# LUMC/kPAL

Hardware: AMD Instinct MI355X
Metric: Gbases/s k-mer counted (k=12, 150bp synthetic) (higher is better)
Workload: dtype int64

## Files before the change

### kpal_amd/csrc/kpal_device.hpp

```cpp
#pragma once
#include <hip/hip_runtime.h>
#include <stdint.h>

namespace kpal {

__host__ __device__ inline uint64_t mix64(uint64_t x)
{
    uint64_t z = x + 0x9E3779B97F4A7C15ULL;
    z = (z ^ (z >> 30)) * 0xBF58476D1CE4E5B9ULL;
    z = (z ^ (z >> 27)) * 0x94D049BB133111EBULL;
    return z ^ (z >> 31);
}

__host__ __device__ inline uint64_t revcomp(uint64_t x, int k)
{
    uint64_t y = ~x;
#if defined(__HIP_DEVICE_COMPILE__)
    y = __brevll(y);
#else
    y = ((y >> 1) & 0x5555555555555555ULL) | ((y & 0x5555555555555555ULL) << 1);
    y = ((y >> 2) & 0x3333333333333333ULL) | ((y & 0x3333333333333333ULL) << 2);
    y = ((y >> 4) & 0x0F0F0F0F0F0F0F0FULL) | ((y & 0x0F0F0F0F0F0F0F0FULL) << 4);
    y = ((y >> 8) & 0x00FF00FF00FF00FFULL) | ((y & 0x00FF00FF00FF00FFULL) << 8);
    y = ((y >> 16) & 0x0000FFFF0000FFFFULL) | ((y & 0x0000FFFF0000FFFFULL) << 16);
    y = (y >> 32) | (y << 32);
#endif
    y = ((y >> 1) & 0x5555555555555555ULL) | ((y & 0x5555555555555555ULL) << 1);
    return y >> (64 - 2 * k);
}

__device__ __forceinline__ void classify4(uint32_t w, uint32_t &t, uint32_t &nz)
{
    t = ((w >> 1) ^ (w >> 2)) & 0x03030303u;
    const uint32_t expect = __builtin_amdgcn_perm(0u, 0x54474341u , t);
    const uint32_t x = (w & 0xDFDFDFDFu) ^ expect;
    nz = (((x & 0x7F7F7F7Fu) + 0x7F7F7F7Fu) | x) & 0x80808080u;
}

template <int SH>
__device__ __forceinline__ uint32_t shl_or(uint32_t a, uint32_t b)
{
    uint32_t r;
    asm("v_lshl_or_b32 %0, %1, %2, %3" : "=v"(r) : "v"(a), "n"(SH), "v"(b));
    return r;
}

__device__ __forceinline__ uint32_t codes_to_top_byte(uint32_t t)
{
    const uint32_t x = shl_or<10>(t, t);
    return shl_or<20>(x, x);
}

__device__ __forceinline__ uint32_t flags_to_top_byte(uint32_t m)
{
    const uint32_t x = shl_or<9>(m, m);
    return shl_or<18>(x, x);
}

__device__ __forceinline__ void encode4(uint32_t w, uint32_t &code8, uint32_t &bad4)
{
    uint32_t t, nz;
    classify4(w, t, nz);
    code8 = codes_to_top_byte(t) >> 24;
    bad4 = flags_to_top_byte(nz >> 7) >> 24;
}

struct Chunk {
    uint32_t codes;
    uint32_t bad;
};

__device__ __forceinline__ Chunk encode16(uint4 v)
{
    uint32_t t0, t1, t2, t3, z0, z1, z2, z3;
    classify4(v.x, t0, z0);
    classify4(v.y, t1, z1);
    classify4(v.z, t2, z2);
    classify4(v.w, t3, z3);
    Chunk r;
#if defined(KPAL_ENCODE_SHIFTS)
    const uint32_t c0 = codes_to_top_byte(t0), c1 = codes_to_top_byte(t1), c2 = codes_to_top_byte(t2), c3 = codes_to_top_byte(t3);
    const uint32_t c01 = __builtin_amdgcn_perm(c0, c1, 0x07030000u);
    const uint32_t c23 = __builtin_amdgcn_perm(c2, c3, 0x07030000u);
    const uint32_t f01 = flags_to_top_byte((z0 >> 3) | (z1 >> 7));
    const uint32_t f23 = flags_to_top_byte((z2 >> 3) | (z3 >> 7));
    r.codes = __builtin_amdgcn_perm(c01, c23, 0x07060302u);
    r.bad = __builtin_amdgcn_perm(f01, f23, 0x0c0c0703u);
#else
    constexpr uint32_t kDigits = 0x01041040u;
    const uint32_t d0 = __builtin_amdgcn_udot4(t0, kDigits, 0u, false), d1 = __builtin_amdgcn_udot4(t1, kDigits, 0u, false);
    const uint32_t d2 = __builtin_amdgcn_udot4(t2, kDigits, 0u, false), d3 = __builtin_amdgcn_udot4(t3, kDigits, 0u, false);
    r.codes = (d0 << 24) | ((d1 << 16) | ((d2 << 8) | d3));
    constexpr uint32_t kHigh = 0x10204080u, kLow = 0x01020408u;
    const uint32_t f01 = __builtin_amdgcn_udot4(z1, kLow, __builtin_amdgcn_udot4(z0, kHigh, 0u, false), false);
    const uint32_t f23 = __builtin_amdgcn_udot4(z3, kLow, __builtin_amdgcn_udot4(z2, kHigh, 0u, false), false);
    r.bad = (f01 << 1) | (f23 >> 7);
#endif
    return r;
}

struct Span {
    const uint4 *base;
    uint64_t lo;
    uint64_t hi;
    uint64_t emit_from;
    uint64_t nchunks;
};

__device__ __forceinline__ uint4 fetch_chunk(const Span &s, int64_t c)
{
    if (c < 0 || (uint64_t)c >= s.nchunks) return make_uint4(0u, 0u, 0u, 0u);
    return s.base[c];
}

__device__ __forceinline__ void range_fix(const Span &s, int64_t c, Chunk &r)
{
    if (c < 0 || (uint64_t)c >= s.nchunks) {
        r.codes = 0;
        r.bad = 0xFFFFu;
        return;
    }
    const uint64_t p0 = (uint64_t)c * 16;
    if (p0 < s.lo || p0 + 16 > s.hi) {
        const uint32_t a = s.lo > p0 ? (uint32_t)(s.lo - p0) : 0u;
        const uint32_t b = s.hi < p0 + 16 ? (uint32_t)(s.hi > p0 ? s.hi - p0 : 0) : 16u;
        const uint32_t in_range = (a < b) ? (((1u << (16 - a)) - 1u) & ~((1u << (16 - b)) - 1u)) : 0u;
        r.bad |= ~in_range & 0xFFFFu;
    }
}

__device__ __forceinline__ Chunk load_chunk(const Span &s, int64_t c)
{
    Chunk r = encode16(fetch_chunk(s, c));
    range_fix(s, c, r);
    return r;
}

template <int K>
__device__ __forceinline__ uint32_t emit_mask(uint32_t prev_bad, uint32_t cur_bad)
{
    uint32_t b = (prev_bad << 16) | cur_bad;
    uint32_t s = b;
    int have = 1;
#pragma unroll
    for (int step = 1; step < 32; step <<= 1) {
        if (have * 2 <= K) {
            s |= s >> have;
            have *= 2;
        }
    }
    if (have < K) s |= s >> (K - have);
    return ~s & 0xFFFFu;
}

__device__ __forceinline__ uint32_t emit_mask_rt(int k, uint32_t prev_bad, uint32_t cur_bad)
{
    uint32_t b = (prev_bad << 16) | cur_bad;
    uint32_t s = b;
    int have = 1;
    while (have * 2 <= k) {
        s |= s >> have;
        have *= 2;
    }
    if (have < k) s |= s >> (k - have);
    return ~s & 0xFFFFu;
}

__device__ __forceinline__ uint32_t emit_from_mask(const Span &s, int64_t c)
{
    const uint64_t p0 = (uint64_t)c * 16;
    if (s.emit_from <= p0) return 0xFFFFu;
    if (s.emit_from >= p0 + 16) return 0u;
    return (1u << (16 - (uint32_t)(s.emit_from - p0))) - 1u;
}

__device__ __forceinline__ uint32_t from_left_lane(uint32_t v, uint32_t lane0_value)
{
    return (uint32_t)__builtin_amdgcn_update_dpp((int)lane0_value, (int)v, 0x138 , 0xF, 0xF, false);
}

template <int K, bool EDGE>
__device__ __forceinline__ void wave_step(const Span &s, int64_t c, Chunk &carry, uint64_t &window,
                                          uint32_t &mask)
{
    Chunk cur;
    if constexpr (EDGE) cur = load_chunk(s, c);
    else cur = encode16(s.base[c]);
    const uint32_t pc = from_left_lane(cur.codes, carry.codes);
    const uint32_t pb = from_left_lane(cur.bad, carry.bad);
    carry.codes = __builtin_amdgcn_readlane(cur.codes, 63);
    carry.bad = __builtin_amdgcn_readlane(cur.bad, 63);
    window = ((uint64_t)pc << 32) | cur.codes;
    mask = emit_mask<K>(pb, cur.bad);
    if constexpr (EDGE) mask &= emit_from_mask(s, c);
}

template <int K>
__device__ __forceinline__ void encode_step(const Span &s, uint64_t step, const uint4 raw, Chunk &carry,
                                            uint64_t &window, uint32_t &mask, bool edge)
{
    const int lane = threadIdx.x & 63;
    const int64_t c = (int64_t)(step * 64 + lane);
    Chunk cur = encode16(raw);
    if (edge) range_fix(s, c, cur);
    const uint32_t pc = from_left_lane(cur.codes, carry.codes);
    const uint32_t pb = from_left_lane(cur.bad, carry.bad);
    carry.codes = __builtin_amdgcn_readlane(cur.codes, 63);
    carry.bad = __builtin_amdgcn_readlane(cur.bad, 63);
    window = ((uint64_t)pc << 32) | cur.codes;
    mask = emit_mask<K>(pb, cur.bad);
    if (edge) mask &= emit_from_mask(s, c);
}

__device__ __forceinline__ bool interior_steps(const Span &s, uint64_t step0, uint64_t step1)
{
    return step0 * 64 >= 1 && (step0 * 64 - 1) * 16 >= s.lo && step1 * 64 * 16 <= s.hi && s.emit_from <= step0 * 64 * 16;
}

template <int K>
__device__ __forceinline__ void encode_step(const Span &s, uint64_t step, const uint4 raw, Chunk &carry,
                                            uint64_t &window, uint32_t &mask)
{
    encode_step<K>(s, step, raw, carry, window, mask, !interior_steps(s, step, step + 1));
}

__device__ __forceinline__ bool interior_range(const Span &s, uint64_t c0, uint64_t c1)
{
    return c0 >= 1 && (c0 - 1) * 16 >= s.lo && c1 * 16 <= s.hi && s.emit_from <= c0 * 16;
}

template <int K>
__device__ __forceinline__ uint32_t kmer_at(uint64_t window, int j)
{
    constexpr uint64_t M = (K >= 16) ? 0xFFFFFFFFULL : ((1ULL << (2 * K)) - 1ULL);
    return (uint32_t)((window >> (2 * (15 - j))) & M);
}

template <int K>
__device__ __forceinline__ void part_step(const Span &s, uint64_t step, Chunk &carry, uint64_t &window, uint32_t &mask)
{
    const int lane = threadIdx.x & 63;
    if (interior_range(s, step * 64, step * 64 + 64)) wave_step<K, false>(s, (int64_t)(step * 64 + lane), carry, window, mask);
    else wave_step<K, true>(s, (int64_t)(step * 64 + lane), carry, window, mask);
}

__device__ __forceinline__ void lds_barrier()
{
    asm volatile("s_waitcnt lgkmcnt(0)\n\ts_barrier" ::: "memory");
}

}
```

### kpal_amd/csrc/quad_kernels.hpp

```cpp
#pragma once
#include <type_traits>

#include "kpal_device.hpp"
#include "quad2_index.hpp"
#include "quad_plan.hpp"

namespace kpal {

constexpr int kQuadSpillCap = 2048;
constexpr int kQuadDummyWords = 4;

template <int K>
struct QuadCfg {
    static_assert(K >= 8 && K <= 16, "quads: k = 8..16");
    static constexpr bool kTwoLevel = K >= 13;
    static constexpr bool kStaged = K >= 12;
    static constexpr int kCoarseBits = kTwoLevel ? 2 * K - 22 : 0;
    static constexpr int kCoarse = 1 << kCoarseBits;
    static constexpr int kRep = kTwoLevel ? (kCoarse >= 256 ? 1 : 256 / kCoarse) : 1;
    static constexpr int kBucketBits = kTwoLevel ? 9 : (K == 12 ? 11 : 9);
    static constexpr int kHistBuckets = 1 << kBucketBits;
    static constexpr int kBuckets = kTwoLevel ? kCoarse * kRep : (1 << kBucketBits);
    static constexpr int kLowBits = kTwoLevel ? 13 : 2 * K - kBucketBits;
    static constexpr int kFormBins = 1 << kLowBits;
    static constexpr int kSlots = kQuadRowWords / kBuckets;
    static constexpr int kRecordBytes = kSlots * 4;
#if defined(KPAL_QUAD_ITEM4)
    static constexpr bool kItem3 = false;
#else
    static constexpr bool kItem3 = !kTwoLevel && K == 12;
#endif
    static constexpr int kItems = kItem3 ? (kSlots / 4) * 5 : kSlots;
#if defined(KPAL_QUAD_NO_PAIR)
    static constexpr bool kPairRows = false;
#else
    static constexpr bool kPairRows = !kTwoLevel && kRecordBytes == 64;
#endif
    static constexpr int kScrBits = (kLowBits - 6) < 4 ? (kLowBits - 6) : 4;
    static constexpr uint64_t kXMask = (1ull << (2 * K + 6)) - 1ull;
    static constexpr uint32_t kLowMask = (1u << kLowBits) - 1u;
    __host__ __device__ static constexpr uint32_t smask(uint32_t t)
    {
        return kScrBits > 0 ? (((t << (kBucketBits - kScrBits)) | t) & (uint32_t)((1 << kBucketBits) - 1)) : 0u;
    }
    __host__ __device__ static constexpr uint32_t smask1(uint32_t t) { return (kCoarseBits > 4 ? ((t << (kCoarseBits - 4)) ^ t) : t) & (uint32_t)(kCoarse - 1); }
};

static_assert(Quad2Index<13>::smask(11) == QuadCfg<13>::smask(11) && Quad2Index<16>::smask(5) == QuadCfg<16>::smask(5) &&
                  Quad2Index<13>::smask1(9) == QuadCfg<13>::smask1(9) && Quad2Index<14>::smask1(13) == QuadCfg<14>::smask1(13) &&
                  Quad2Index<15>::smask1(7) == QuadCfg<15>::smask1(7) && Quad2Index<16>::smask1(15) == QuadCfg<16>::smask1(15) &&
                  Quad2Index<15>::CB == QuadCfg<15>::kCoarseBits &&
                  ((Quad2Index<12>::smask1(13) << 9) | Quad2Index<12>::smask(13)) == QuadCfg<12>::smask(13) &&
                  ((Quad2Index<12>::smask1(6) << 9) | Quad2Index<12>::smask(6)) == QuadCfg<12>::smask(6),
              "quad2_index.hpp restates the scramble masks of QuadCfg");

template <int K>
__device__ __forceinline__ void quad_split(uint64_t x, uint32_t m4, uint32_t lane, uint32_t &row, uint32_t &item)
{
    using C = QuadCfg<K>;
    const uint32_t low = (uint32_t)x & C::kLowMask;
    const uint32_t hi6 = (uint32_t)(x >> (2 * K));
    if constexpr (C::kTwoLevel) {
        const uint32_t fine = ((uint32_t)x >> 13) & 511u;
        const uint32_t coarse = (uint32_t)(x >> 22) & (uint32_t)(C::kCoarse - 1);
        row = (coarse ^ C::smask1(low >> 9)) * C::kRep + (lane & (uint32_t)(C::kRep - 1));
        item = (hi6 << 26) | (fine << 17) | (low << 4) | m4;
    } else {
        const uint32_t b = ((uint32_t)x >> C::kLowBits) & (uint32_t)(C::kBuckets - 1);
        row = b ^ C::smask(low >> (C::kLowBits - C::kScrBits));
        item = (hi6 << (C::kLowBits + 4)) | (low << 4) | m4;
    }
}

template <int K, int LEVEL = 1>
__device__ __forceinline__ uint32_t quad_kmer(uint32_t row, uint32_t item, int i, uint32_t coarse = 0)
{
    using C = QuadCfg<K>;
    uint64_t x;
    if constexpr (LEVEL == 2) {
        const uint32_t low = (item >> 4) & 8191u, hi6 = item >> 17, t = low >> 9;
        x = ((uint64_t)hi6 << (2 * K)) | ((uint64_t)(coarse ^ C::smask1(t)) << 22) | ((uint64_t)(row ^ C::smask(t)) << 13) | low;
    } else if constexpr (C::kTwoLevel) {
        const uint32_t low = (item >> 4) & 8191u, fine = (item >> 17) & 511u, hi6 = item >> 26, t = low >> 9;
        x = ((uint64_t)hi6 << (2 * K)) | ((uint64_t)((row / C::kRep) ^ C::smask1(t)) << 22) | ((uint64_t)fine << 13) | low;
    } else {
        const uint32_t low = (item >> 4) & C::kLowMask;
        const uint32_t hi6 = item >> (C::kLowBits + 4);
        const uint32_t b = row ^ C::smask(low >> (C::kLowBits - C::kScrBits));
        x = ((uint64_t)hi6 << (2 * K)) | ((uint64_t)b << C::kLowBits) | low;
    }
    return (uint32_t)((x >> (6 - 2 * i)) & ((1ull << (2 * K)) - 1ull));
}

struct QuadPacked {
    uint32_t a, b, c;
};
__device__ __forceinline__ QuadPacked quad_pack3(const uint4 &v)
{
    QuadPacked r;
    r.a = v.x | (v.y << 23);
    r.b = (v.y >> 9) | (v.z << 14);
    r.c = (v.z >> 18) | (v.w << 5);
    return r;
}
__device__ __forceinline__ uint4 quad_unpack3(uint32_t a, uint32_t b, uint32_t c)
{
    uint4 v;
    v.x = a & 0x7FFFFFu;
    v.y = __builtin_amdgcn_alignbit(b, a, 23) & 0x7FFFFFu;
    v.z = __builtin_amdgcn_alignbit(c, b, 14) & 0x7FFFFFu;
    v.w = (c >> 5) & 0x7FFFFFu;
    return v;
}

struct QuadSpill {
    uint32_t row, item;
};

struct QuadHot {
    unsigned long long key;
    uint32_t count, pad;
};
constexpr int kQuadHotEntries = 256;

struct TableSink {
    unsigned long long *table;
    unsigned long long *list;
    uint32_t *count;
    uint32_t cap;
    uint32_t *overflow;
};

struct TableOnly {
    unsigned long long *table;
};

__device__ __forceinline__ void sink_add(const TableOnly &sink, uint64_t index, unsigned long long n) { atomicAdd(&sink.table[index], n); }

struct TableSinkRef {
    const TableSink *p;
};

__device__ __forceinline__ void sink_add(const TableSink &sink, uint64_t index, unsigned long long n);
__device__ __forceinline__ void sink_add(const TableSinkRef &ref, uint64_t index, unsigned long long n) { sink_add(*ref.p, index, n); }

__device__ __forceinline__ void sink_add(const TableSink &sink, uint64_t index, unsigned long long n)
{
    if (sink.table) {
        atomicAdd(&sink.table[index], n);
    } else {
        const uint32_t at = atomicAdd(sink.count, 1u);
        if (at < sink.cap) sink.list[at] = ((unsigned long long)index << 32) | (n & 0xFFFFFFFFull);
        else *sink.overflow = 1u;
    }
}

__device__ __forceinline__ uint32_t quad_hot_hash(uint32_t row, uint32_t item)
{
    return ((item >> 4) * 0x9E3779B1u + row * 0x85EBCA6Bu) >> 24;
}

template <typename SINK>
__device__ __attribute__((noinline)) void quad_hot_age(const SINK table, QuadHot *hot)
{
    const QuadHot h = hot[threadIdx.x];
    if (h.key >> 63) {
        if (h.count == h.pad) {
            sink_add(table, (uint64_t)(h.key & 0x7FFFFFFFFFFFFFFFull), (unsigned long long)h.count);
            hot[threadIdx.x] = QuadHot{0ull, 0u, 0u};
        } else {
            hot[threadIdx.x].pad = h.count;
        }
    }
}

template <typename SINK>
__device__ __forceinline__ void quad_kmer_add(const SINK table, QuadHot *hot, uint64_t index, uint32_t n)
{
#if defined(KPAL_AB_DIRECT_NO_TABLE)
    return;
#endif
    const unsigned long long key = (1ull << 63) | (unsigned long long)index;
    const uint32_t h = ((uint32_t)index * 0x9E3779B1u + (uint32_t)(index >> 32)) >> 24;
    bool done = false;
#pragma unroll 1
    for (uint32_t pr = 0; pr < 4u && !done; ++pr) {
        const uint32_t slot = (h + pr) & (uint32_t)(kQuadHotEntries - 1);
        unsigned long long cur = hot[slot].key;
        if (cur == 0ull) {
            cur = atomicCAS(&hot[slot].key, 0ull, key);
            if (cur == 0ull) cur = key;
        }
        if (cur == key) {
            atomicAdd(&hot[slot].count, n);
            done = true;
        }
    }
    if (!done) sink_add(table, index, (unsigned long long)n);
}

template <int K, int LEVEL = 1, typename SINK = TableOnly, bool COUNTED = false, bool KMERS = false>
__device__ __forceinline__ void quad_items_direct_body(bool active, uint32_t row, uint32_t item, const SINK table, QuadHot *hot, uint32_t coarse = 0,
                                                       uint32_t cnt = 1u)
{
    const uint32_t mult = COUNTED ? cnt : 1u;
    const int lane = threadIdx.x & 63;
    auto kmer_add = [&](uint64_t index, uint32_t n) {
        if constexpr (KMERS) quad_kmer_add<SINK>(table, hot, index, n);
        else sink_add(table, index, (unsigned long long)n);
    };
    auto to_table = [&](uint32_t r, uint32_t it, uint32_t n) {
#pragma unroll
        for (int i = 0; i < 4; ++i)
            if ((it >> (3 - i)) & 1u) sink_add(table, quad_kmer<K, LEVEL>(r, it, i, coarse), (unsigned long long)n);
    };
    unsigned long long todo = __builtin_amdgcn_ballot_w64(active);
    for (int round = 0; round < 8 && todo; ++round) {
        const int src = __ffsll((long long)todo) - 1;
        const uint32_t hot_row = (uint32_t)__builtin_amdgcn_readlane(row, src);
        const uint32_t hot_item = (uint32_t)__builtin_amdgcn_readlane(item, src);
        const unsigned long long same = __builtin_amdgcn_ballot_w64(active && row == hot_row && item == hot_item) & todo;
        uint32_t n = (uint32_t)__popcll(same);
        if constexpr (COUNTED) {
            n = 0;
#pragma unroll
            for (uint32_t v = 1; v <= 4u; ++v) n += v * (uint32_t)__popcll(same & __builtin_amdgcn_ballot_w64(cnt == v));
        }
        const unsigned long long key = ((unsigned long long)hot_row << 32) | hot_item;
        const uint32_t slot = (quad_hot_hash(hot_row, hot_item) + (uint32_t)(lane & 3)) & (uint32_t)(kQuadHotEntries - 1);
        const unsigned long long seen = lane < 4 ? hot[slot].key : ~0ull;
        const unsigned long long hit = __builtin_amdgcn_ballot_w64(seen == key);
        if (hit) {
            if (lane == __ffsll((long long)hit) - 1) atomicAdd(&hot[slot].count, n);
        } else {
            const unsigned long long free_slots = __builtin_amdgcn_ballot_w64(seen == 0ull);
            bool placed = false;
            if (n >= 2u && free_slots) {
                const int who = __ffsll((long long)free_slots) - 1;
                const unsigned long long old = lane == who ? atomicCAS(&hot[slot].key, 0ull, key) : 1ull;
                placed = __builtin_amdgcn_ballot_w64(lane == who && (old == 0ull || old == key)) != 0ull;
                if (placed && lane == who) atomicAdd(&hot[slot].count, n);
            }
            if constexpr (KMERS) {
                if (!placed && lane < 4 && ((hot_item >> (3 - lane)) & 1u)) kmer_add(quad_kmer<K, LEVEL>(hot_row, hot_item, lane, coarse), n);
            } else {
                if (!placed && lane == src) to_table(hot_row, hot_item, n);
            }
        }
        todo &= ~same;
    }
    if ((todo >> lane) & 1ull) {
        const unsigned long long key = ((unsigned long long)row << 32) | item;
        const uint32_t h = quad_hot_hash(row, item);
        bool done = false;
#pragma unroll
        for (int pr = 0; pr < 4 && !done; ++pr) {
            const uint32_t slot = (h + (uint32_t)pr) & (uint32_t)(kQuadHotEntries - 1);
            if (hot[slot].key == key) {
                atomicAdd(&hot[slot].count, mult);
                done = true;
            }
        }
        if (!done) to_table(row, item, mult);
    }
}

template <int K, int LEVEL = 1, typename SINK = TableOnly, bool KM = false>
__device__ __attribute__((noinline)) void quad_items_direct(bool active, uint32_t row, uint32_t item, const SINK table, QuadHot *hot, uint32_t coarse = 0)
{
    quad_items_direct_body<K, LEVEL, SINK, false, KM>(active, row, item, table, hot, coarse);
}

template <int K, typename SINK>
__device__ __attribute__((noinline)) void quad_items_direct_counted(uint32_t cnt, uint32_t row, uint32_t item, const SINK table, QuadHot *hot)
{
    quad_items_direct_body<K, 1, SINK, true, true>(cnt != 0u, row, item, table, hot, 0u, cnt);
}

template <int K, bool DIRECT = false, int LEVEL = 1, int N = 4, typename SINK = TableOnly, bool KM = false>
__device__ __forceinline__ uint32_t quad_place(uint32_t *rows, uint32_t *pos, QuadSpill *spill, uint32_t *spill_n, uint32_t cap,
                                               const uint32_t (&row)[N], const uint32_t (&item)[N], const SINK &table,
                                               QuadHot *hot, uint32_t coarse = 0)
{
    using C = typename std::conditional<LEVEL == 2, QuadCfg<11>, QuadCfg<K>>::type;
    constexpr uint32_t RB = (uint32_t)C::kSlots * 4u;
    constexpr bool ITEM3 = LEVEL == 1 && C::kItem3;
    uint32_t riders = 0;
    uint32_t off[N];
#pragma unroll
    for (int q = 0; q < N; ++q) off[q] = atomicAdd(&pos[row[q]], (item[q] & 15u) ? 4u : 0u);
    uint32_t over = 0;
#pragma unroll
    for (int q = 0; q < N; ++q) {
        const bool counted = (item[q] & 15u) != 0u;
        if constexpr (ITEM3) {
            const bool normal = off[q] < RB;
            const bool rider = !normal && off[q] < RB + RB / 4;
            if (counted && normal) atomicOr(reinterpret_cast<uint32_t *>(reinterpret_cast<char *>(rows) + row[q] * RB + off[q]), item[q]);
            riders |= (counted && rider) ? (1u << q) : 0u;
            over |= (counted && !normal && !rider) ? (1u << q) : 0u;
        } else {
            const bool fits = off[q] < RB;
            const uint32_t at = row[q] * RB + off[q];
            *reinterpret_cast<uint32_t *>(reinterpret_cast<char *>(rows) + ((counted && fits) ? at : (uint32_t)kQuadRowWords * 4u)) = item[q];
            over |= (counted && !fits) ? (1u << q) : 0u;
        }
    }
#if defined(KPAL_AB_SCATTER_NO_RIDER)
    riders = 0;
#endif
#if defined(KPAL_AB_SCATTER_NO_SPILL)
    over = 0;
#endif
    if constexpr (ITEM3) {
        if (__any(riders != 0u)) {
#pragma unroll
            for (int q = 0; q < N; ++q)
                if ((riders >> q) & 1u) {
                    uint32_t *p = reinterpret_cast<uint32_t *>(reinterpret_cast<char *>(rows) + row[q] * RB + (off[q] - RB) * 4u);
#if defined(KPAL_AB_RIDER_OR)
                    atomicOr(p, item[q] << 24);
                    atomicOr(p + 1, (item[q] << 16) & 0xFF000000u);
                    atomicOr(p + 2, (item[q] << 8) & 0xFF000000u);
#else
                    reinterpret_cast<unsigned char *>(p)[3] = (unsigned char)item[q];
                    reinterpret_cast<unsigned char *>(p)[7] = (unsigned char)(item[q] >> 8);
                    reinterpret_cast<unsigned char *>(p)[11] = (unsigned char)(item[q] >> 16);
#endif
                }
        }
    }
    if (__builtin_expect(__any(over != 0u), 0)) {
#if defined(KPAL_QUAD_NO_CARRY)
        constexpr bool direct = true;
#else
        constexpr bool direct = DIRECT;
#endif
#if defined(KPAL_AB_SPILL_LANE)
        if constexpr (!direct) {
            uint32_t at[N];
#pragma unroll
            for (int q = 0; q < N; ++q) at[q] = cap;
            if (over) {
#pragma unroll
                for (int q = 0; q < N; ++q)
                    if ((over >> q) & 1u) at[q] = atomicAdd(spill_n, 1u);
            }
            uint32_t unlisted = 0;
#pragma unroll
            for (int q = 0; q < N; ++q) {
                const bool ov = (over >> q) & 1u;
                if (ov && at[q] < cap) spill[at[q]] = QuadSpill{row[q], item[q]};
                unlisted |= (ov && at[q] >= cap) ? (1u << q) : 0u;
            }
            if (__builtin_expect(__any(unlisted != 0u), 0)) {
#pragma unroll
                for (int q = 0; q < N; ++q)
                    if (__any((unlisted >> q) & 1u)) quad_items_direct<K, LEVEL, SINK, KM>((unlisted >> q) & 1u, row[q], item[q], table, hot, coarse);
            }
            return over;
        }
#endif
        uint32_t base = 0;
        bool list_full = true;
        unsigned long long bq[N];
#pragma unroll
        for (int q = 0; q < N; ++q) bq[q] = __builtin_amdgcn_ballot_w64((over >> q) & 1u);
        if constexpr (!direct) {
            uint32_t total = 0;
#pragma unroll
            for (int q = 0; q < N; ++q) total += (uint32_t)__popcll(bq[q]);
            uint32_t got = 0;
            if ((threadIdx.x & 63u) == 0u) got = atomicAdd(spill_n, total);
            base = (uint32_t)__builtin_amdgcn_readfirstlane((int)got);
            list_full = base + total > cap;
        }
#pragma unroll
        for (int q = 0; q < N; ++q) {
            if (bq[q] == 0ull) continue;
            const bool ov = (over >> q) & 1u;
            bool listed = false;
            if constexpr (!direct) {
                const unsigned long long b = bq[q];
                const uint32_t at = base + __builtin_amdgcn_mbcnt_hi((uint32_t)(b >> 32), __builtin_amdgcn_mbcnt_lo((uint32_t)b, 0u));
                listed = ov && at < cap;
                if (listed) spill[at] = QuadSpill{row[q], item[q]};
                base += (uint32_t)__popcll(b);
            }
            if (list_full && __any(ov && !listed)) quad_items_direct<K, LEVEL, SINK, KM>(ov && !listed, row[q], item[q], table, hot, coarse);
        }
    }
    return over;
}

template <int K, int CARRY, int LEVEL = 1, typename SINK = TableOnly, bool KM = false>
__device__ __forceinline__ void quad_place_carried(uint32_t *rows, uint32_t *pos, QuadSpill *spill, uint32_t *spill_n, uint32_t cap,
                                                   const uint32_t (&carry_row)[CARRY], uint32_t (&carry_item)[CARRY],
                                                   const SINK &table, QuadHot *hot, uint32_t coarse = 0)
{
#pragma unroll
    for (int c = 0; c < CARRY; ++c) {
        const uint32_t r1[1] = {carry_row[c]};
        const uint32_t i1[1] = {carry_item[c]};
        if (__any(carry_item[c] != 0u)) {
            if (quad_place<K, true, LEVEL, 1, SINK, KM>(rows, pos, spill, spill_n, cap, r1, i1, table, hot, coarse) & 1u) carry_item[c] = 0;
        }
    }
}

template <int CARRY, int THREADS>
__device__ __forceinline__ void quad_take_carried(const QuadSpill *spill, uint32_t n, uint32_t (&carry_row)[CARRY],
                                                  uint32_t (&carry_item)[CARRY])
{
#pragma unroll
    for (int c = 0; c < CARRY; ++c) {
        const uint32_t e = threadIdx.x + (uint32_t)c * THREADS;
        carry_item[c] = 0;
        if (e < n) {
            carry_row[c] = spill[e].row;
            carry_item[c] = spill[e].item;
        }
    }
}

template <int STEPS>
__device__ __forceinline__ void quad_tile_priority(int st)
{
#if !defined(KPAL_QUAD_NO_PRIO)
    const int level = st * 4 / STEPS;
    if (st == 0 || level != (st - 1) * 4 / STEPS) {
        switch (level) {
        case 0: __builtin_amdgcn_s_setprio(3); break;
        case 1: __builtin_amdgcn_s_setprio(2); break;
        case 2: __builtin_amdgcn_s_setprio(1); break;
        default: __builtin_amdgcn_s_setprio(0); break;
        }
    }
#endif
}

__device__ __forceinline__ void quad_note_spill(uint32_t *__restrict__ error, uint32_t appended, uint32_t cap)
{
    if (threadIdx.x == 0 && appended) {
        atomicAdd(error + 2, min(appended, cap));
        if (appended > cap) atomicAdd(error + 3, appended - cap);
    }
}

template <int K>
__global__ __launch_bounds__(512) void quad_sample_kernel(Span s, uint64_t stride_steps, uint32_t steps, uint32_t *__restrict__ load)
{
    using C = QuadCfg<K>;
    constexpr int NFINE = C::kTwoLevel ? 512 : 0;
    constexpr int NCNT = C::kBuckets + NFINE + 1;
    __shared__ uint32_t cnt[NCNT];
    for (int i = threadIdx.x; i < NCNT; i += blockDim.x) cnt[i] = 0;
    __syncthreads();
    const int wave = threadIdx.x >> 6;
    const uint64_t total_steps = (s.nchunks + 63) / 64;
    const uint64_t first = (uint64_t)blockIdx.x * stride_steps + (uint64_t)wave * steps;
    if (first < total_steps) {
        Chunk carry = load_chunk(s, (int64_t)(first * 64) - 1);
        for (uint32_t st = 0; st < steps && first + st < total_steps; ++st) {
            uint64_t window;
            uint32_t mask;
            part_step<K>(s, first + st, carry, window, mask);
            uint32_t row[4], item[4];
#pragma unroll
            for (int q = 0; q < 4; ++q) {
                const uint64_t x = (window >> (24 - 8 * q)) & C::kXMask;
                quad_split<K>(x, (mask >> (12 - 4 * q)) & 15u, threadIdx.x & 63u, row[q], item[q]);
            }
            {
                const bool c01 = item[1] == item[0] && row[1] == row[0] && (item[1] & 15u) == 15u;
                const bool c23 = item[3] == item[2] && row[3] == row[2] && (item[3] & 15u) == 15u;
                const unsigned long long cand = __builtin_amdgcn_ballot_w64(c01 || c23);
                if (cand) {
                    const int src = __ffsll((long long)cand) - 1;
                    const uint32_t hot_item = (uint32_t)__builtin_amdgcn_readlane(c01 ? item[1] : item[3], src);
                    const uint32_t hot_row = (uint32_t)__builtin_amdgcn_readlane(c01 ? row[1] : row[3], src);
                    uint32_t n = 0;
#pragma unroll
                    for (int q = 0; q < 4; ++q) {
                        const bool m = item[q] == hot_item && row[q] == hot_row;
                        n += m ? 1u : 0u;
                        item[q] = m ? 0u : item[q];
                    }
                    if (n) atomicAdd(&cnt[NCNT - 1], n);
                }
            }
#pragma unroll
            for (int q = 0; q < 4; ++q) {
                atomicAdd(&cnt[row[q]], (item[q] & 15u) ? 1u : 0u);
                if constexpr (C::kTwoLevel) {
                    const uint32_t fine_row = ((item[q] >> 17) & 511u) ^ QuadCfg<11>::smask(((item[q] >> 4) & 8191u) >> 9);
                    atomicAdd(&cnt[C::kBuckets + fine_row], (item[q] & 15u) ? 1u : 0u);
                }
            }
        }
    }
    __syncthreads();
    for (int i = threadIdx.x; i < NCNT; i += blockDim.x)
        if (cnt[i]) atomicAdd(&load[i], cnt[i]);
}

__device__ __forceinline__ uint4 fetch_wave_step(const Span &s, uint64_t step, uint32_t lane16)
{
    if ((step + 1) * 64 <= s.nchunks)
        return *reinterpret_cast<const uint4 *>(reinterpret_cast<const char *>(s.base + step * 64) + lane16);
    return fetch_chunk(s, (int64_t)(step * 64 + (lane16 >> 4)));
}


template <int K, int WAVES, int STEPS, int DEPTH, typename SINK = TableOnly, bool REPEAT = false>
__global__ __launch_bounds__(WAVES * 64) void quad_scatter_kernel(Span s, uint64_t tiles_per_block, uint32_t *__restrict__ pool,
                                                                  uint32_t rounds_cap, uint32_t *__restrict__ nrounds,
                                                                  uint32_t *__restrict__ error, SINK sink_arg)
{
    using C = QuadCfg<K>;
    constexpr bool kLists = std::is_same<SINK, TableSink>::value;
    constexpr int S = C::kSlots, NB = C::kBuckets;
    constexpr int THREADS = WAVES * 64;
    constexpr int kQuadTileSteps = WAVES * STEPS;
    constexpr int CARRY = kQuadSpillCap / THREADS;
    constexpr uint32_t CAP = CARRY * THREADS;
    static_assert((WAVES == 8 || WAVES == 16) && STEPS % DEPTH == 0, "tile shape");
    __shared__ __attribute__((aligned(16))) uint32_t rows[kQuadRowWords + kQuadDummyWords];
    __shared__ __attribute__((aligned(16))) uint32_t pos[NB];
    __shared__ QuadSpill spill[kQuadSpillCap];
    __shared__ uint32_t spill_cnt[2];
    __shared__ QuadHot hot[kQuadHotEntries];
    __shared__ uint32_t direct_n;
    __shared__ TableSink sink_lds;
    using SINK2 = typename std::conditional<kLists, TableSinkRef, SINK>::type;
    SINK2 table;
    if constexpr (kLists) {
        if (threadIdx.x == 0) {
            TableSink t = sink_arg;
            if (t.list) {
                t.list += (size_t)blockIdx.x * t.cap;
                t.count = &direct_n;
            }
            sink_lds = t;
            direct_n = 0;
        }
        table = TableSinkRef{&sink_lds};
    } else {
        table = sink_arg;
    }
    const int wave = __builtin_amdgcn_readfirstlane((int)(threadIdx.x >> 6)), lane = threadIdx.x & 63;
    const uint32_t lane16 = (uint32_t)lane * 16u;
    for (int i = threadIdx.x; i < kQuadRowWords + kQuadDummyWords; i += THREADS) rows[i] = 0;
    for (int i = threadIdx.x; i < NB; i += THREADS) pos[i] = 0;
    for (int i = threadIdx.x; i < kQuadHotEntries; i += THREADS) hot[i] = QuadHot{0ull, 0u, 0u};
    if (threadIdx.x == 0) {
        spill_cnt[0] = 0;
        spill_cnt[1] = 0;
    }
    __syncthreads();
    const uint64_t total_steps = (s.nchunks + 63) / 64;
    auto tile_step = [&](uint64_t j) -> uint64_t { return ((j * gridDim.x + blockIdx.x) * WAVES + (uint64_t)wave) * STEPS; };
    auto tile_exists = [&](uint64_t j) -> bool { return j < tiles_per_block && (j * gridDim.x + blockIdx.x) * (uint64_t)kQuadTileSteps < total_steps; };
    uint4 raw[DEPTH];
    uint4 rawh;
    {
        const uint64_t f = tile_step(0);
#pragma unroll
        for (int st = 0; st < DEPTH; ++st) raw[st] = fetch_wave_step(s, f + st, lane16);
        rawh = fetch_chunk(s, (int64_t)(f * 64) - 1);
    }
    uint32_t round = 0;
    uint32_t carry_row[CARRY], carry_item[CARRY];
#pragma unroll
    for (int c = 0; c < CARRY; ++c) carry_row[c] = carry_item[c] = 0;
    constexpr int LPR = S / 4;
    constexpr int FI = kQuadRowWords / 4 / THREADS;
    static_assert(THREADS % LPR == 0, "a record is written by one wave");
    uint4 rec[FI];
    bool have_rec = false;
    constexpr int PAIR = C::kPairRows ? 2 : 1;
    static_assert((THREADS / LPR) % PAIR == 0, "row pairs are written by one instruction");
    const uint64_t row_bytes = (uint64_t)gridDim.x * rounds_cap * (uint64_t)(S * 4 * PAIR);
    const uint32_t thread_off = (uint32_t)((uint64_t)(threadIdx.x / (LPR * PAIR)) * row_bytes) + (threadIdx.x % (LPR * PAIR)) * 16u;
    auto store_rec = [&](int i) {
#if defined(KPAL_AB_POOL_FILL)
        if (i % 7 == 6) return;
#endif
        uint32_t o = thread_off;
        asm volatile("" : "+v"(o));
        const uint64_t sc = (uint64_t)(i * (THREADS / (LPR * PAIR))) * row_bytes + ((uint64_t)blockIdx.x * rounds_cap + (round - 1u)) * (uint64_t)(S * 4 * PAIR);
#if defined(KPAL_QUAD_NT)
        uint32_t *q = reinterpret_cast<uint32_t *>(reinterpret_cast<char *>(pool) + sc + o);
        __builtin_nontemporal_store(rec[i].x, q);
        __builtin_nontemporal_store(rec[i].y, q + 1);
        __builtin_nontemporal_store(rec[i].z, q + 2);
        __builtin_nontemporal_store(rec[i].w, q + 3);
#elif defined(KPAL_AB_SCATTER_NO_STORE)
        asm volatile("" ::"v"(rec[i].x ^ rec[i].y ^ rec[i].z ^ rec[i].w), "v"(o), "s"((uint32_t)sc));
#else
        *reinterpret_cast<uint4 *>(reinterpret_cast<char *>(pool) + sc + o) = rec[i];
#endif
    };
    auto store_rec_at = [&](int i, const uint4 &v) {
        const uint64_t sc = (uint64_t)i * (uint64_t)(THREADS / (LPR * PAIR)) * row_bytes + ((uint64_t)blockIdx.x * rounds_cap + (round - 1u)) * (uint64_t)(S * 4 * PAIR);
        *reinterpret_cast<uint4 *>(reinterpret_cast<char *>(pool) + sc + thread_off) = v;
    };
    for (uint64_t j = 0; tile_exists(j); ++j) {
        const uint64_t first = tile_step(j);
        const bool more = tile_exists(j + 1);
        const uint64_t fnext = tile_step(j + 1);
        const bool edge = !interior_steps(s, first, first + STEPS);
        const bool next_inside = more && (fnext + STEPS) * 64 <= s.nchunks;
        uint32_t *spill_n = &spill_cnt[j & 1];
        quad_place_carried<K, CARRY, 1, SINK2, REPEAT>(rows, pos, spill, spill_n, CAP, carry_row, carry_item, table, hot);
        Chunk carry = encode16(rawh);
        range_fix(s, (int64_t)(first * 64) - 1, carry);
        if (more) rawh = fetch_chunk(s, (int64_t)(fnext * 64) - 1);
#pragma unroll
        for (int st = 0; st < STEPS; ++st) {
            uint64_t window;
            uint32_t mask;
            quad_tile_priority<STEPS>(st);
            encode_step<K>(s, first + st, raw[st % DEPTH], carry, window, mask, edge);
            if (have_rec) {
#pragma unroll
                for (int i = st * (FI / STEPS); i < (st + 1) * (FI / STEPS); ++i) store_rec(i);
            }
            {
                uint32_t l16 = lane16;
                asm volatile("" : "+v"(l16));
                if (st + DEPTH < STEPS) raw[st % DEPTH] = fetch_wave_step(s, first + st + DEPTH, l16);
                else if (next_inside) raw[st % DEPTH] = *reinterpret_cast<const uint4 *>(reinterpret_cast<const char *>(s.base + (fnext + (st + DEPTH - STEPS)) * 64) + l16);
                else if (more) raw[st % DEPTH] = fetch_chunk(s, (int64_t)((fnext + (st + DEPTH - STEPS)) * 64 + (l16 >> 4)));
            }
            uint32_t row[4], item[4];
#pragma unroll
            for (int q = 0; q < 4; ++q) {
                const uint64_t x = (window >> (24 - 8 * q)) & C::kXMask;
                quad_split<K>(x, (mask >> (12 - 4 * q)) & 15u, (uint32_t)lane, row[q], item[q]);
            }
            bool place = true;
            if constexpr (REPEAT) {
                if (__builtin_expect(__any(item[1] == item[0] || item[3] == item[2]), 0)) {
                    const bool c01 = item[1] == item[0] && row[1] == row[0] && (item[1] & 15u) == 15u;
                    const bool c23 = item[3] == item[2] && row[3] == row[2] && (item[3] & 15u) == 15u;
                    const unsigned long long cand = __builtin_amdgcn_ballot_w64(c01 || c23);
                    if (cand) {
                        const int src = __ffsll((long long)cand) - 1;
                        const uint32_t hot_item = (uint32_t)__builtin_amdgcn_readlane(c01 ? item[1] : item[3], src);
                        const uint32_t hot_row = (uint32_t)__builtin_amdgcn_readlane(c01 ? row[1] : row[3], src);
                        uint32_t cnt = 0;
#pragma unroll
                        for (int q = 0; q < 4; ++q) {
                            const bool m = item[q] == hot_item && row[q] == hot_row;
                            cnt += m ? 1u : 0u;
                            item[q] = m ? 0u : item[q];
                        }
                        quad_items_direct_counted<K, SINK2>(cnt, hot_row, hot_item, table, hot);
                        place = __any((item[0] | item[1] | item[2] | item[3]) != 0u);
                    }
                }
            }
#if defined(KPAL_AB_SCATTER_NO_PLACE)
            asm volatile("" ::"v"(row[0] ^ row[1] ^ row[2] ^ row[3] ^ item[0] ^ item[1] ^ item[2] ^ item[3]));
#else
            if (place) quad_place<K, false, 1, 4, SINK2, REPEAT>(rows, pos, spill, spill_n, CAP, row, item, table, hot);
#endif
        }
        have_rec = false;
        quad_tile_priority<1>(0);
        lds_barrier();
        const uint32_t spilled = min(*spill_n, CAP);
        quad_note_spill(error, *spill_n, CAP);
        if (threadIdx.x == 0) spill_cnt[(j & 1) ^ 1] = 0;
        if constexpr (REPEAT) {
            if ((j & 3u) == 3u && threadIdx.x < (uint32_t)kQuadHotEntries) quad_hot_age<SINK2>(table, hot);
        }
        quad_take_carried<CARRY, THREADS>(spill, spilled, carry_row, carry_item);
        {
            const uint4 zero4 = make_uint4(0u, 0u, 0u, 0u);
            uint4 *rv = reinterpret_cast<uint4 *>(rows);
#pragma unroll
            for (int i = 0; i < FI; ++i) {
                const uint4 v = rv[threadIdx.x + (uint32_t)i * THREADS];
                rec[i].x = v.x;
                rec[i].y = v.y;
                rec[i].z = v.z;
                rec[i].w = v.w;
                rv[threadIdx.x + (uint32_t)i * THREADS] = zero4;
            }
            for (int i = threadIdx.x * 4; i < NB; i += THREADS * 4) *reinterpret_cast<uint4 *>(&pos[i]) = zero4;
        }
        if (round >= rounds_cap) {
            if (threadIdx.x == 0) *error = 2u;
        } else {
            have_rec = true;
            ++round;
#pragma unroll
            for (int i = STEPS * (FI / STEPS); i < FI; ++i) store_rec(i);
        }
        lds_barrier();
    }
    if (have_rec) {
#pragma unroll
        for (int i = 0; i < STEPS * (FI / STEPS); ++i) store_rec(i);
    }
    if constexpr (kLists) {
        if (round > 0u && round < rounds_cap) {
            static_assert(!C::kItem3, "plain four-byte slots");
#pragma unroll
            for (int c = 0; c < CARRY; ++c)
                if (carry_item[c]) {
                    const uint32_t off = atomicAdd(&pos[carry_row[c]], 4u);
                    if (off < (uint32_t)S * 4u) {
                        *reinterpret_cast<uint32_t *>(reinterpret_cast<char *>(rows) + carry_row[c] * (uint32_t)(S * 4) + off) = carry_item[c];
                        carry_item[c] = 0;
                    }
                }
            lds_barrier();
            const uint4 *rv = reinterpret_cast<const uint4 *>(rows);
            ++round;
#pragma unroll 1
            for (int h = 0; h < FI; h += 4) {
#pragma unroll
                for (int i = 0; i < 4; ++i) rec[i] = rv[threadIdx.x + (uint32_t)(h + i) * THREADS];
#pragma unroll
                for (int i = 0; i < 4; ++i) store_rec_at(h + i, rec[i]);
            }
        }
    }
    if (threadIdx.x == 0) nrounds[blockIdx.x] = min(round, rounds_cap);
#pragma unroll
    for (int c = 0; c < CARRY; ++c) quad_items_direct_body<K, 1, SINK2>(carry_item[c] != 0u, carry_row[c], carry_item[c], table, hot);
    __syncthreads();
    uint32_t used = 0;
    for (int i = threadIdx.x; i < kQuadHotEntries; i += THREADS) {
        const QuadHot h = hot[i];
        if (h.key && h.count) {
            ++used;
            if (h.key >> 63) {
                sink_add(table, (uint64_t)(h.key & 0x7FFFFFFFFFFFFFFFull), (unsigned long long)h.count);
                continue;
            }
            const uint32_t r = (uint32_t)(h.key >> 32), it = (uint32_t)h.key;
#pragma unroll
            for (int q = 0; q < 4; ++q)
                if ((it >> (3 - q)) & 1u) sink_add(table, quad_kmer<K>(r, it, q), (unsigned long long)h.count);
        }
    }
    if (used) atomicAdd(error + 1, used);
    if constexpr (kLists) {
        if (sink_arg.list) {
            __syncthreads();
            if (threadIdx.x == 0) sink_arg.count[blockIdx.x] = min(direct_n, sink_arg.cap);
        }
    }
}

template <int K, int WAVES, int STEPS, bool KM = false>
__global__ __launch_bounds__(WAVES * 64) void quad2_scatter_kernel(const uint32_t *__restrict__ pool1, const uint32_t *__restrict__ nrounds1,
                                                            uint32_t G1, uint32_t rounds_cap1, uint32_t upw, uint32_t tiles_per_block,
                                                            uint32_t *__restrict__ pool2, uint32_t rounds_cap2,
                                                            uint32_t *__restrict__ nrounds2, uint32_t *__restrict__ error,
                                                            TableSink sink_arg)
{
    using C1 = QuadCfg<K>;
    using C = QuadCfg<11>;
    constexpr int S = C::kSlots, NB = C::kBuckets, S1 = C1::kSlots;
    constexpr int THREADS = WAVES * 64;
    static_assert(WAVES == 8 || WAVES == 16, "tile shape");
    constexpr int CARRY = kQuadSpillCap / THREADS;
    constexpr uint32_t CAP = CARRY * THREADS;
    __shared__ __attribute__((aligned(16))) uint32_t rows[kQuadRowWords + kQuadDummyWords];
    __shared__ __attribute__((aligned(16))) uint32_t pos[NB];
    __shared__ QuadSpill spill[kQuadSpillCap];
    __shared__ uint32_t spill_cnt[2];
    __shared__ QuadHot hot[kQuadHotEntries];
    __shared__ uint32_t nr1[256];
    __shared__ uint32_t direct_n;
    __shared__ TableSink sink_lds;
    const uint32_t wg_linear = blockIdx.y * gridDim.x + blockIdx.x;
    if (threadIdx.x == 0) {
        TableSink t = sink_arg;
        if (t.list) {
            t.list += (size_t)wg_linear * t.cap;
            t.count = &direct_n;
        }
        sink_lds = t;
        direct_n = 0;
    }
    const TableSinkRef table = {&sink_lds};
    const int wave = __builtin_amdgcn_readfirstlane((int)(threadIdx.x >> 6)), lane = threadIdx.x & 63;
    const uint32_t coarse = blockIdx.y;
    for (int i = threadIdx.x; i < kQuadRowWords + kQuadDummyWords; i += THREADS) rows[i] = 0;
    for (int i = threadIdx.x; i < NB; i += THREADS) pos[i] = 0;
    for (int i = threadIdx.x; i < kQuadHotEntries; i += THREADS) hot[i] = QuadHot{0ull, 0u, 0u};
    for (uint32_t i = threadIdx.x; i < 256u; i += THREADS) nr1[i] = i < G1 ? nrounds1[i] : 0u;
    if (threadIdx.x == 0) {
        spill_cnt[0] = 0;
        spill_cnt[1] = 0;
    }
    __syncthreads();
    const uint32_t units = (uint32_t)C1::kRep * G1;
    const uint32_t u0 = blockIdx.x * upw, u1 = min(u0 + upw, units);
    const uint32_t unit_cap = rounds_cap1 * (uint32_t)(S1 * 4);
    const uint32_t stream = (u1 > u0 ? u1 - u0 : 0u) * unit_cap;
    const uint32_t lane16 = (uint32_t)lane * 16u;
    uint64_t nx_p = 0;
    uint32_t nx_g1 = 0, nx_rl = 0, nx_off = 0;
    auto seek = [&](uint64_t j) {
        nx_p = ((j * WAVES + (uint64_t)wave) * STEPS) * 1024ull;
        if (nx_p < (uint64_t)stream) {
            const uint32_t ul = (uint32_t)nx_p / unit_cap;
            nx_off = (uint32_t)nx_p - ul * unit_cap;
            const uint32_t u = u0 + ul;
            nx_rl = u / G1;
            nx_g1 = u - nx_rl * G1;
        }
    };
    auto fetch_next = [&]() -> uint4 {
        uint4 v = make_uint4(0u, 0u, 0u, 0u);
        if (nx_p < (uint64_t)stream) {
            const uint32_t written = nr1[nx_g1] * (uint32_t)(S1 * 4);
            if (nx_off + lane16 < written) {
                const char *src = reinterpret_cast<const char *>(pool1) +
                                  ((uint64_t)((coarse * C1::kRep + nx_rl) * G1 + nx_g1) * rounds_cap1) * (uint64_t)(S1 * 4) + nx_off;
                v = *reinterpret_cast<const uint4 *>(src + lane16);
            }
            nx_p += 1024;
            nx_off += 1024;
            if (nx_off >= unit_cap) {
                nx_off = 0;
                if (++nx_g1 == G1) {
                    nx_g1 = 0;
                    ++nx_rl;
                }
            }
        }
        return v;
    };
    uint4 raw[STEPS];
    seek(0);
#pragma unroll
    for (int st = 0; st < STEPS; ++st) raw[st] = fetch_next();
    uint32_t round = 0;
    uint32_t carry_row[CARRY], carry_item[CARRY];
#pragma unroll
    for (int c = 0; c < CARRY; ++c) carry_row[c] = carry_item[c] = 0;
    constexpr int LPR = S / 4;
    constexpr int NVEC = NB * LPR;
    constexpr int FI = NVEC / THREADS;
    constexpr int DEFER = FI / STEPS;
    static_assert(S == 64 && LPR == 16, "packed records of 64 items");
    QuadPacked rec[FI];
    bool have_rec = false;
    const uint32_t wg = coarse * gridDim.x + blockIdx.x;
    constexpr uint32_t PIECE = 2u * (uint32_t)kQuadPackedRecordBytes;
    const uint64_t row_bytes = (uint64_t)gridDim.x * rounds_cap2 * (uint64_t)PIECE;
    const uint32_t thread_off = (uint32_t)((uint64_t)(threadIdx.x / (2 * LPR)) * row_bytes) + (threadIdx.x % (2 * LPR)) * 12u;
    auto store_rec = [&](int i) {
        uint32_t o = thread_off;
        asm volatile("" : "+v"(o));
        const uint64_t sc = ((uint64_t)coarse * (NB / 2) + (uint64_t)(i * (THREADS / (2 * LPR)))) * row_bytes + ((uint64_t)blockIdx.x * rounds_cap2 + (round - 1u)) * (uint64_t)PIECE;
        *reinterpret_cast<QuadPacked *>(reinterpret_cast<char *>(pool2) + sc + o) = rec[i];
    };
    auto store_rec_at = [&](int i, const QuadPacked &v) {
        const uint64_t sc = ((uint64_t)coarse * (NB / 2) + (uint64_t)i * (uint64_t)(THREADS / (2 * LPR))) * row_bytes + ((uint64_t)blockIdx.x * rounds_cap2 + (round - 1u)) * (uint64_t)PIECE;
        *reinterpret_cast<QuadPacked *>(reinterpret_cast<char *>(pool2) + sc + thread_off) = v;
    };
    const uint64_t tile_bytes = (uint64_t)WAVES * STEPS * 1024;
    for (uint64_t j = 0; j < tiles_per_block && j * tile_bytes < (uint64_t)stream; ++j) {
        const bool more = j + 1 < tiles_per_block && (j + 1) * tile_bytes < (uint64_t)stream;
        uint32_t *spill_n = &spill_cnt[j & 1];
        quad_place_carried<K, CARRY, 2, TableSinkRef, KM>(rows, pos, spill, spill_n, CAP, carry_row, carry_item, table, hot, coarse);
        if (more) seek(j + 1);
#pragma unroll
        for (int st = 0; st < STEPS; ++st) {
            quad_tile_priority<STEPS>(st);
            const uint4 v = raw[st];
            const uint32_t it[4] = {v.x, v.y, v.z, v.w};
            uint32_t row[4], item[4];
#pragma unroll
            for (int q = 0; q < 4; ++q) {
                const uint32_t t = ((it[q] >> 4) & 8191u) >> 9;
                row[q] = ((it[q] >> 17) & 511u) ^ C::smask(t);
                item[q] = ((it[q] >> 26) << 17) | (it[q] & 0x1FFFFu);
            }
            asm volatile("" ::"v"(row[0]), "v"(item[0]));
            if (have_rec) {
#pragma unroll
                for (int i = st * DEFER; i < (st + 1) * DEFER; ++i) store_rec(i);
            }
            if (more) raw[st] = fetch_next();
            quad_place<K, false, 2, 4, TableSinkRef, KM>(rows, pos, spill, spill_n, CAP, row, item, table, hot, coarse);
        }
        have_rec = false;
        quad_tile_priority<1>(0);
        lds_barrier();
        const uint32_t spilled = min(*spill_n, CAP);
        quad_note_spill(error, *spill_n, CAP);
        if (threadIdx.x == 0) spill_cnt[(j & 1) ^ 1] = 0;
        if constexpr (KM) {
            if ((j & 3u) == 3u && threadIdx.x < (uint32_t)kQuadHotEntries) quad_hot_age<TableSinkRef>(table, hot);
        }
        quad_take_carried<CARRY, THREADS>(spill, spilled, carry_row, carry_item);
        {
            const uint4 zero4 = make_uint4(0u, 0u, 0u, 0u);
            uint4 *rv = reinterpret_cast<uint4 *>(rows);
#pragma unroll
            for (int i = 0; i < FI; ++i) {
                const uint4 v = rv[threadIdx.x + (uint32_t)i * THREADS];
                rec[i] = quad_pack3(v);
                rv[threadIdx.x + (uint32_t)i * THREADS] = zero4;
            }
            for (int i = threadIdx.x * 4; i < NB; i += THREADS * 4) *reinterpret_cast<uint4 *>(&pos[i]) = zero4;
        }
        if (round >= rounds_cap2) {
            if (threadIdx.x == 0) *error = 3u;
        } else {
            have_rec = true;
            ++round;
#pragma unroll
            for (int i = STEPS * DEFER; i < FI; ++i) store_rec(i);
        }
        lds_barrier();
    }
    if (have_rec) {
#pragma unroll
        for (int i = 0; i < STEPS * DEFER; ++i) store_rec(i);
    }
    {
        if (round > 0u && round < rounds_cap2) {
#pragma unroll
            for (int c = 0; c < CARRY; ++c)
                if (carry_item[c]) {
                    const uint32_t off = atomicAdd(&pos[carry_row[c]], 4u);
                    if (off < (uint32_t)S * 4u) {
                        *reinterpret_cast<uint32_t *>(reinterpret_cast<char *>(rows) + carry_row[c] * (uint32_t)(S * 4) + off) = carry_item[c];
                        carry_item[c] = 0;
                    }
                }
            lds_barrier();
            const uint4 *rv = reinterpret_cast<const uint4 *>(rows);
            ++round;
#pragma unroll 1
            for (int h = 0; h < FI; h += 4) {
#pragma unroll
                for (int i = 0; i < 4; ++i) rec[i] = quad_pack3(rv[threadIdx.x + (uint32_t)(h + i) * THREADS]);
#pragma unroll
                for (int i = 0; i < 4; ++i) store_rec_at(h + i, rec[i]);
            }
        }
    }
    if (threadIdx.x == 0) nrounds2[wg] = min(round, rounds_cap2);
#pragma unroll
    for (int c = 0; c < CARRY; ++c) quad_items_direct<K, 2, TableSinkRef, KM>(carry_item[c] != 0u, carry_row[c], carry_item[c], table, hot, coarse);
    __syncthreads();
    for (int i = threadIdx.x; i < kQuadHotEntries; i += THREADS) {
        const QuadHot h = hot[i];
        if (h.key && h.count) {
            if (h.key >> 63) {
                sink_add(table, (uint64_t)(h.key & 0x7FFFFFFFFFFFFFFFull), (unsigned long long)h.count);
// ... 437 lines not shown
```

Measured before the change: 1533.

## Trim classify ops, use ballot votes, drop rider vote, strength-reduce store addressing

```diff
diff --git a/kpal_amd/csrc/kpal_device.hpp b/kpal_amd/csrc/kpal_device.hpp
--- a/kpal_amd/csrc/kpal_device.hpp
+++ b/kpal_amd/csrc/kpal_device.hpp
@@ -33,8 +33,22 @@
 {
     t = ((w >> 1) ^ (w >> 2)) & 0x03030303u;
     const uint32_t expect = __builtin_amdgcn_perm(0u, 0x54474341u , t);
+#if defined(KPAL_AB_CLASSIFY_OLD)
     const uint32_t x = (w & 0xDFDFDFDFu) ^ expect;
     nz = (((x & 0x7F7F7F7Fu) + 0x7F7F7F7Fu) | x) & 0x80808080u;
+#else
+    const uint32_t x7 = (w & 0x5F5F5F5Fu) ^ expect;
+    nz = ((x7 + 0x7F7F7F7Fu) | w) & 0x80808080u;
+#endif
+}
+
+__device__ __forceinline__ bool wave_any(bool p)
+{
+#if defined(KPAL_AB_VOTE_ANY)
+    return __any(p);
+#else
+    return __builtin_amdgcn_ballot_w64(p) != 0ull;
+#endif
 }
 
 template <int SH>
diff --git a/kpal_amd/csrc/quad_kernels.hpp b/kpal_amd/csrc/quad_kernels.hpp
--- a/kpal_amd/csrc/quad_kernels.hpp
+++ b/kpal_amd/csrc/quad_kernels.hpp
@@ -313,7 +313,10 @@
     over = 0;
 #endif
     if constexpr (ITEM3) {
-        if (__any(riders != 0u)) {
+#if defined(KPAL_AB_RIDER_VOTE)
+        if (wave_any(riders != 0u))
+#endif
+        {
 #pragma unroll
             for (int q = 0; q < N; ++q)
                 if ((riders >> q) & 1u) {
@@ -330,7 +333,7 @@
                 }
         }
     }
-    if (__builtin_expect(__any(over != 0u), 0)) {
+    if (__builtin_expect(wave_any(over != 0u), 0)) {
 #if defined(KPAL_QUAD_NO_CARRY)
         constexpr bool direct = true;
 #else
@@ -353,10 +356,10 @@
                 if (ov && at[q] < cap) spill[at[q]] = QuadSpill{row[q], item[q]};
                 unlisted |= (ov && at[q] >= cap) ? (1u << q) : 0u;
             }
-            if (__builtin_expect(__any(unlisted != 0u), 0)) {
+            if (__builtin_expect(wave_any(unlisted != 0u), 0)) {
 #pragma unroll
                 for (int q = 0; q < N; ++q)
-                    if (__any((unlisted >> q) & 1u)) quad_items_direct<K, LEVEL, SINK, KM>((unlisted >> q) & 1u, row[q], item[q], table, hot, coarse);
+                    if (wave_any((unlisted >> q) & 1u)) quad_items_direct<K, LEVEL, SINK, KM>((unlisted >> q) & 1u, row[q], item[q], table, hot, coarse);
             }
             return over;
         }
@@ -387,7 +390,7 @@
                 if (listed) spill[at] = QuadSpill{row[q], item[q]};
                 base += (uint32_t)__popcll(b);
             }
-            if (list_full && __any(ov && !listed)) quad_items_direct<K, LEVEL, SINK, KM>(ov && !listed, row[q], item[q], table, hot, coarse);
+            if (list_full && wave_any(ov && !listed)) quad_items_direct<K, LEVEL, SINK, KM>(ov && !listed, row[q], item[q], table, hot, coarse);
         }
     }
     return over;
@@ -402,7 +405,7 @@
     for (int c = 0; c < CARRY; ++c) {
         const uint32_t r1[1] = {carry_row[c]};
         const uint32_t i1[1] = {carry_item[c]};
-        if (__any(carry_item[c] != 0u)) {
+        if (wave_any(carry_item[c] != 0u)) {
             if (quad_place<K, true, LEVEL, 1, SINK, KM>(rows, pos, spill, spill_n, cap, r1, i1, table, hot, coarse) & 1u) carry_item[c] = 0;
         }
     }
@@ -582,13 +585,24 @@
     static_assert((THREADS / LPR) % PAIR == 0, "row pairs are written by one instruction");
     const uint64_t row_bytes = (uint64_t)gridDim.x * rounds_cap * (uint64_t)(S * 4 * PAIR);
     const uint32_t thread_off = (uint32_t)((uint64_t)(threadIdx.x / (LPR * PAIR)) * row_bytes) + (threadIdx.x % (LPR * PAIR)) * 16u;
+    const uint64_t rec_stride = (uint64_t)(THREADS / (LPR * PAIR)) * row_bytes;
+    uint64_t rec_run = 0;
+    auto rec_round_base = [&]() -> uint64_t { return ((uint64_t)blockIdx.x * rounds_cap + (round - 1u)) * (uint64_t)(S * 4 * PAIR); };
     auto store_rec = [&](int i) {
+        uint32_t o = thread_off;
+        asm volatile("" : "+v"(o));
+#if defined(KPAL_AB_STORE_BASE_MUL)
+        const uint64_t sc = (uint64_t)(i * (THREADS / (LPR * PAIR))) * row_bytes + rec_round_base();
+#else
+        if (i == 0) rec_run = rec_round_base();
+        else if (i == STEPS * (FI / STEPS)) rec_run = rec_round_base() + (uint64_t)i * rec_stride;
+        asm volatile("" : "+s"(rec_run));
+        const uint64_t sc = rec_run;
+        rec_run += rec_stride;
+#endif
 #if defined(KPAL_AB_POOL_FILL)
         if (i % 7 == 6) return;
 #endif
-        uint32_t o = thread_off;
-        asm volatile("" : "+v"(o));
-        const uint64_t sc = (uint64_t)(i * (THREADS / (LPR * PAIR))) * row_bytes + ((uint64_t)blockIdx.x * rounds_cap + (round - 1u)) * (uint64_t)(S * 4 * PAIR);
 #if defined(KPAL_QUAD_NT)
         uint32_t *q = reinterpret_cast<uint32_t *>(reinterpret_cast<char *>(pool) + sc + o);
         __builtin_nontemporal_store(rec[i].x, q);
@@ -641,7 +655,7 @@
             }
             bool place = true;
             if constexpr (REPEAT) {
-                if (__builtin_expect(__any(item[1] == item[0] || item[3] == item[2]), 0)) {
+                if (__builtin_expect(wave_any(item[1] == item[0]) || wave_any(item[3] == item[2]), 0)) {
                     const bool c01 = item[1] == item[0] && row[1] == row[0] && (item[1] & 15u) == 15u;
                     const bool c23 = item[3] == item[2] && row[3] == row[2] && (item[3] & 15u) == 15u;
                     const unsigned long long cand = __builtin_amdgcn_ballot_w64(c01 || c23);
@@ -657,7 +671,7 @@
                             item[q] = m ? 0u : item[q];
                         }
                         quad_items_direct_counted<K, SINK2>(cnt, hot_row, hot_item, table, hot);
-                        place = __any((item[0] | item[1] | item[2] | item[3]) != 0u);
+                        place = wave_any((item[0] | item[1] | item[2] | item[3]) != 0u);
                     }
                 }
             }
```

After: 1541 (median of 6 runs). About the same (+0.5%).
